# Vincentqyw/image-matching-webui

Measured on AMD Instinct MI355X. Metric: image-pairs/sec @640x480 SuperPoint+LightGlue, higher is better.
Workload: dtype f32 via 3xf16 split MFMA, f32 accumulate; P.V of LightGlue's cross blocks in two products (audited per block: layer error <= 7.1e-6, score error <= 4.7e-5, profiles/r05_lab_attention_mix.txt)

## Files before the change

image-matching-webui_amd/csrc/gemm_wreg.hip:

```cpp
#include <stdlib.h>

#include "gemm.h"
#include "gemm_tile.h"

#define WR_BN 256
#ifdef WR_LAB
__device__ int wr_lab_flags = 0;
#define WR_FLAGS (__builtin_amdgcn_readfirstlane(wr_lab_flags))
#else
#define WR_FLAGS 0
#endif
#define WR_F_NOSTORE 1
#define WR_F_ONETILE 2
#define WR_F_NOEPI 4
#define WR_F_NOWLOAD 8
#define WR_F_NOXLOAD 16
#define WR_F_NOSTORE_V 32
#define WR_F_NOSTORE_QK 64
#define WR_F_STAGGER(f) (((f) >> 8) & 255)
#define WR_STG_ROW 68
#define WR_STG_TROW 36
#define WR_WAVE_LDS 9216

typedef unsigned int u32x4_t __attribute__((ext_vector_type(4)));
__device__ __forceinline__ const void* wr_uniform_ptr(const void* p) {
    const size_t v = (size_t)p;
    const unsigned lo32 = (unsigned)__builtin_amdgcn_readfirstlane((int)(unsigned)(v & 0xffffffffu));
    const unsigned hi32 = (unsigned)__builtin_amdgcn_readfirstlane((int)(unsigned)(v >> 32));
    return (const void*)((size_t)lo32 | ((size_t)hi32 << 32));
}
__device__ __forceinline__ void wr_wave_fence() {
    __builtin_amdgcn_s_waitcnt(0xc07f);
    __builtin_amdgcn_wave_barrier();
}

template <int EPI, bool SINGLE, bool PIPE = true, int MT = 4>
__global__ __launch_bounds__(256, 2) void gemm_wreg_kernel(GemmP p) {
    __shared__ uint4 smem[(4 * WR_WAVE_LDS) / 16];
    char* sm = reinterpret_cast<char*>(smem);
    const int tid = threadIdx.x;
    const int lane = tid & 63, wid = tid >> 6;
    const int lo = lane & 31, hi = lane >> 5;
    TileCtx c;
    if (!gemm_tile_setup(p, c, WR_BN, 32 * MT)) return;
    const float* A = p.A + (size_t)c.z * p.a_bs;
    const float wsc = p.wscale ? p.wscale[c.wsel] : 1.0f;
    const int labf = WR_FLAGS;
    if (WR_F_STAGGER(labf) != 0 && (int)blockIdx.x >= p.st_nct && (int)blockIdx.x < 4 * p.st_nct)
        for (int i = 0; i < WR_F_STAGGER(labf) * ((int)blockIdx.x / p.st_nct); ++i) __builtin_amdgcn_s_sleep(16);
    const int nkt = (labf & WR_F_ONETILE) ? 1 : p.K >> 5, nks = 2 * nkt;

    f32x16 acc[2][MT];
#pragma unroll
    for (int n = 0; n < 2; ++n)
#pragma unroll
        for (int m = 0; m < MT; ++m)
#pragma unroll
            for (int r = 0; r < 16; ++r) acc[n][m][r] = 0.0f;

    const int g = tid & 3;
    const int rl0 = tid >> 2, rl1 = 64 + (tid >> 2);
    const bool st0 = MT >= 2 || rl0 < 32, st1 = MT == 4;
    const int wo0 = (((g >> 1) * 4 + (rl0 >> 5)) * 64 + (g & 1) * 32 + ((rl0 & 31) ^ (2 * g))) * 16;
    const int wo1 = (((g >> 1) * 4 + (rl1 >> 5)) * 64 + (g & 1) * 32 + ((rl1 & 31) ^ (2 * g))) * 16;
    const float* pa0 = A + (size_t)min(c.row0 + (st0 ? rl0 : 0), c.M - 1) * p.lda + g * 8;
    const float* pa1 = A + (size_t)min(c.row0 + (st1 ? rl1 : 0), c.M - 1) * p.lda + g * 8;
    bool lnc = false;
    float mu0 = 0.f, mu1 = 0.f;
    if constexpr (EPI == EPI_QKV_VIT || EPI == EPI_CONV) {
        lnc = p.ln_stats != nullptr;
        if (lnc) {
            mu0 = p.ln_stats[2 * (size_t)min(c.row0 + (st0 ? rl0 : 0), c.M - 1)];
            mu1 = p.ln_stats[2 * (size_t)min(c.row0 + (st1 ? rl1 : 0), c.M - 1)];
        }
    }
    f32x4 xa0, xb0, xa1, xb1;
    auto issue = [&](int kt) __attribute__((always_inline)) {
        if (st0) {
            xa0 = *reinterpret_cast<const f32x4*>(pa0 + kt * 32);
            xb0 = *reinterpret_cast<const f32x4*>(pa0 + kt * 32 + 4);
        }
        if (st1) {
            xa1 = *reinterpret_cast<const f32x4*>(pa1 + kt * 32);
            xb1 = *reinterpret_cast<const f32x4*>(pa1 + kt * 32 + 4);
        }
    };
    auto store = [&](int stg) __attribute__((always_inline)) {
        uint4 h, l;
        if constexpr (EPI == EPI_QKV_VIT || EPI == EPI_CONV) {
            if (lnc) {
                xa0 -= mu0;
                xb0 -= mu0;
                xa1 -= mu1;
                xb1 -= mu1;
            }
        }
        if constexpr (SINGLE) {
            if (st0) *reinterpret_cast<uint4*>(sm + stg * 16384 + wo0) = half8_rtn(__builtin_bit_cast(float4, xa0), __builtin_bit_cast(float4, xb0));
            if (st1) *reinterpret_cast<uint4*>(sm + stg * 16384 + wo1) = half8_rtn(__builtin_bit_cast(float4, xa1), __builtin_bit_cast(float4, xb1));
            return;
        }
        if (st0) {
            split8(__builtin_bit_cast(float4, xa0), __builtin_bit_cast(float4, xb0), h, l);
            *reinterpret_cast<uint4*>(sm + stg * 16384 + wo0) = h;
            if constexpr (!SINGLE) *reinterpret_cast<uint4*>(sm + stg * 16384 + 8192 + wo0) = l;
        }
        if (st1) {
            split8(__builtin_bit_cast(float4, xa1), __builtin_bit_cast(float4, xb1), h, l);
            *reinterpret_cast<uint4*>(sm + stg * 16384 + wo1) = h;
            if constexpr (!SINGLE) *reinterpret_cast<uint4*>(sm + stg * 16384 + 8192 + wo1) = l;
        }
    };
    const int nfr = (p.N + 31) >> 5;
    const size_t plane_bytes = (size_t)nfr * 32 * p.K * 2;
    const __amdgpu_buffer_rsrc_t rWh =
        __builtin_amdgcn_make_buffer_rsrc(const_cast<void*>(wr_uniform_ptr(p.Wh + (size_t)c.wsel * p.w_stride)), 0, (unsigned)plane_bytes, 0x00020000);
    const __amdgpu_buffer_rsrc_t rWl =
        __builtin_amdgcn_make_buffer_rsrc(const_cast<void*>(wr_uniform_ptr(p.Wl + (size_t)c.wsel * p.w_stride)), 0, (unsigned)plane_bytes, 0x00020000);
    unsigned wof[2];
#pragma unroll
    for (int n = 0; n < 2; ++n) {
        const int nf = min((c.col0 >> 5) + 2 * wid + n, nfr - 1);
        wof[n] = (unsigned)((nf * (p.K >> 4)) * 64 + lane) * 16u;
    }
    uint4 wc[2][2], wn[2][2];
    auto loadw = [&](int s, uint4(&w)[2][2]) __attribute__((always_inline)) {
#pragma unroll
        for (int n = 0; n < 2; ++n) {
            const u32x4_t vh = __builtin_amdgcn_raw_buffer_load_b128(rWh, wof[n], (unsigned)s * 1024u, 0);
            w[n][0] = make_uint4(vh.x, vh.y, vh.z, vh.w);
            if constexpr (!SINGLE) {
                const u32x4_t vl = __builtin_amdgcn_raw_buffer_load_b128(rWl, wof[n], (unsigned)s * 1024u, 0);
                w[n][1] = make_uint4(vl.x, vl.y, vl.z, vl.w);
            }
        }
    };
    auto kstep = [&](int stg, int ks, uint4(&w)[2][2]) __attribute__((always_inline)) {
        const int apos = (hi * 32 + (lo ^ (2 * (2 * ks + hi)))) * 16;
#pragma unroll
        for (int mh = 0; mh < (MT + 1) / 2; ++mh) {
            constexpr int MH = MT >= 2 ? 2 : 1;
            uint4 ah[MH], al[MH];
#pragma unroll
            for (int m = 0; m < MH; ++m) {
                const int fo = stg * 16384 + (ks * 4 + 2 * mh + m) * 1024 + apos;
                ah[m] = *reinterpret_cast<const uint4*>(sm + fo);
                if constexpr (!SINGLE) al[m] = *reinterpret_cast<const uint4*>(sm + fo + 8192);
            }
#pragma unroll
            for (int n = 0; n < 2; ++n)
#pragma unroll
                for (int m = 0; m < MH; ++m) {
                    if constexpr (!SINGLE) {
                        acc[n][2 * mh + m] = mfma16(w[n][0], al[m], acc[n][2 * mh + m]);
                        acc[n][2 * mh + m] = mfma16(w[n][1], ah[m], acc[n][2 * mh + m]);
                    }
                    acc[n][2 * mh + m] = mfma16(w[n][0], ah[m], acc[n][2 * mh + m]);
                }
            if constexpr (PIPE) {
                if (mh == 0) __builtin_amdgcn_sched_barrier(0);
            }
        }
    };

    if constexpr (PIPE) {
        uint4 w0[2][2], w1[2][2], w2[2][2];
        issue(0);
        loadw(0, w0);
        if (nks > 1) loadw(1, w1);
        store(0);
        if (nkt > 1) issue(1);
        __syncthreads();
#define WR_TILE(KT, WA, WB, WC)                                  \
    {                                                            \
        const int kt_ = (KT), stg_ = kt_ & 1, s_ = 2 * kt_;      \
        if (s_ + 2 < nks && !(labf & WR_F_NOWLOAD)) loadw(s_ + 2, WC); \
        __builtin_amdgcn_sched_barrier(0);                       \
        kstep(stg_, 0, WA);                                      \
        __builtin_amdgcn_sched_barrier(0);                       \
        if (kt_ + 1 < nkt && !(labf & WR_F_NOXLOAD)) {           \
            store(stg_ ^ 1);                                     \
            if (kt_ + 2 < nkt) issue(kt_ + 2);                   \
        }                                                        \
        if (s_ + 3 < nks && !(labf & WR_F_NOWLOAD)) loadw(s_ + 3, WA); \
        __builtin_amdgcn_sched_barrier(0);                       \
        kstep(stg_, 1, WB);                                      \
        __syncthreads();                                         \
    }
        int kt = 0;
#pragma unroll 1
        for (; kt + 3 <= nkt; kt += 3) {
            WR_TILE(kt, w0, w1, w2)
            WR_TILE(kt + 1, w2, w0, w1)
            WR_TILE(kt + 2, w1, w2, w0)
        }
        if (kt < nkt) WR_TILE(kt, w0, w1, w2)
        if (kt + 1 < nkt) WR_TILE(kt + 1, w2, w0, w1)
#undef WR_TILE
    } else {
    issue(0);
    loadw(0, wc);
    store(0);
    if (nkt > 1) issue(1);
    __syncthreads();
#pragma unroll 1
    for (int kt = 0; kt < nkt; ++kt) {
        const int stg = kt & 1;
        loadw(2 * kt + 1, wn);
        kstep(stg, 0, wc);
        if (kt + 1 < nkt) {
            store(stg ^ 1);
            if (kt + 2 < nkt) issue(kt + 2);
            loadw(2 * kt + 2, wc);
        }
        kstep(stg, 1, wn);
        __syncthreads();
    }
    }

    float* st = reinterpret_cast<float*>(sm + wid * WR_WAVE_LDS);
    const int fw0 = c.col0 + 64 * wid;
    if (fw0 >= c.N) return;
    if (labf & WR_F_NOEPI) {
        if (acc[0][0][0] == 12345.678f) p.C[0] = acc[1][MT - 1][3];
        return;
    }
    bool do_store = !(labf & WR_F_NOSTORE);
    auto park_rows = [&](int m) __attribute__((always_inline)) {
#pragma unroll
        for (int n = 0; n < 2; ++n)
#pragma unroll
            for (int q = 0; q < 4; ++q)
                *reinterpret_cast<float4*>(st + lo * WR_STG_ROW + 32 * n + 8 * q + 4 * hi) =
                    make_float4(acc[n][m][4 * q + 0] * wsc, acc[n][m][4 * q + 1] * wsc, acc[n][m][4 * q + 2] * wsc, acc[n][m][4 * q + 3] * wsc);
    };
    if constexpr (EPI == EPI_QKV || EPI == EPI_CROSS || EPI == EPI_QKV_VIT) {
        const int CW = p.heads * 64;
        const int t = fw0 / CW, hd = (fw0 - t * CW) >> 6;
        float* dst;
        bool vt, rope, scale;
        if (EPI == EPI_QKV || EPI == EPI_QKV_VIT) {
            const int role = t + (EPI == EPI_QKV_VIT ? p.role0 : 0);
            dst = (role == 0) ? p.Q : (role == 1) ? p.Kt : p.V;
            vt = (role == 2);
            rope = (role < 2);
            scale = (role == 0);
        } else {
            dst = (t == 0) ? p.Q : p.V;
            vt = (t == 1);
            rope = false;
            scale = (t == 0);
        }
        unsigned short* d16 = reinterpret_cast<unsigned short*>(dst);
        if ((labf & WR_F_NOSTORE_V) && vt) do_store = false;
        if ((labf & WR_F_NOSTORE_QK) && !vt) do_store = false;
        const int R = p.rows_per_seq;
        const int i0 = c.row0 - c.seq * R;
        if (EPI == EPI_QKV_VIT && !vt) {
            const int tab0 = i0 + (p.rope_seq_row0 ? p.rope_seq_row0[c.seq] : 0);
            const int d0 = (lane & 7) * 8, dp = d0 ^ 16;
            const bool first = (d0 & 16) == 0;
            const int ti = (d0 >> 5) * 16 + (d0 & 8);
            float4 ba = make_float4(0.f, 0.f, 0.f, 0.f), bb = ba, pa = ba, pb = ba;
            if (c.bias != nullptr) {
                ba = *reinterpret_cast<const float4*>(c.bias + fw0 + d0);
                bb = *reinterpret_cast<const float4*>(c.bias + fw0 + d0 + 4);
                pa = *reinterpret_cast<const float4*>(c.bias + fw0 + dp);
                pb = *reinterpret_cast<const float4*>(c.bias + fw0 + dp + 4);
            }
#pragma unroll
            for (int m = 0; m < MT; ++m) {
                float4 tc[4][2], ts[4][2];
#pragma unroll
                for (int pass = 0; pass < 4; ++pass) {
                    const size_t ir = (size_t)(tab0 + 32 * m + pass * 8 + (lane >> 3)) * 32 + ti;
                    tc[pass][0] = *reinterpret_cast<const float4*>(p.rope_cos + ir);
                    tc[pass][1] = *reinterpret_cast<const float4*>(p.rope_cos + ir + 4);
                    ts[pass][0] = *reinterpret_cast<const float4*>(p.rope_sin + ir);
                    ts[pass][1] = *reinterpret_cast<const float4*>(p.rope_sin + ir + 4);
                }
                park_rows(m);
                wr_wave_fence();
#pragma unroll
                for (int pass = 0; pass < 4; ++pass) {
                    const int tl = pass * 8 + (lane >> 3);
                    const float4 va = *reinterpret_cast<const float4*>(st + tl * WR_STG_ROW + d0);
                    const float4 vb = *reinterpret_cast<const float4*>(st + tl * WR_STG_ROW + d0 + 4);
                    const float4 wa = *reinterpret_cast<const float4*>(st + tl * WR_STG_ROW + dp);
                    const float4 wb = *reinterpret_cast<const float4*>(st + tl * WR_STG_ROW + dp + 4);
                    float mine[8] = {va.x + ba.x, va.y + ba.y, va.z + ba.z, va.w + ba.w, vb.x + bb.x, vb.y + bb.y, vb.z + bb.z, vb.w + bb.w};
                    float part[8] = {wa.x + pa.x, wa.y + pa.y, wa.z + pa.z, wa.w + pa.w, wb.x + pb.x, wb.y + pb.y, wb.z + pb.z, wb.w + pb.w};
                    if (lnc) {
                        const float2 mr = *reinterpret_cast<const float2*>(p.ln_stats + 2 * (size_t)(c.row0 + 32 * m + tl));
                        const float xa[8] = {va.x, va.y, va.z, va.w, vb.x, vb.y, vb.z, vb.w}, xp[8] = {wa.x, wa.y, wa.z, wa.w, wb.x, wb.y, wb.z, wb.w};
                        const float ba8[8] = {ba.x, ba.y, ba.z, ba.w, bb.x, bb.y, bb.z, bb.w}, pa8[8] = {pa.x, pa.y, pa.z, pa.w, pb.x, pb.y, pb.z, pb.w};
#pragma unroll
                        for (int j = 0; j < 8; ++j) {
                            mine[j] = mr.y * xa[j] + ba8[j];
                            part[j] = mr.y * xp[j] + pa8[j];
                        }
                    }
                    const float cw[8] = {tc[pass][0].x, tc[pass][0].y, tc[pass][0].z, tc[pass][0].w, tc[pass][1].x, tc[pass][1].y, tc[pass][1].z, tc[pass][1].w};
                    const float ss[8] = {ts[pass][0].x, ts[pass][0].y, ts[pass][0].z, ts[pass][0].w, ts[pass][1].x, ts[pass][1].y, ts[pass][1].z, ts[pass][1].w};
                    float v[8];
#pragma unroll
                    for (int j = 0; j < 8; ++j) {
                        float x = mine[j], y = part[j];
                        asm volatile("" : "+v"(x), "+v"(y));
                        const float r = first ? __builtin_fmaf(x, cw[j], -(y * ss[j])) : __builtin_fmaf(x, cw[j], y * ss[j]);
                        v[j] = scale ? r * p.alpha : r;
                    }
                    uint4 hv, lv;
                    split8(make_float4(v[0], v[1], v[2], v[3]), make_float4(v[4], v[5], v[6], v[7]), hv, lv);
                    unsigned short* o = d16 + (((size_t)c.seq * p.heads + hd) * R + i0 + 32 * m + tl) * 64 + d0;
                    if (do_store) {
                        *reinterpret_cast<uint4*>(o) = hv;
                        *reinterpret_cast<uint4*>(o + p.plane_halves) = lv;
                    }
                }
                wr_wave_fence();
            }
        } else if (!vt) {
            const int d0 = (lane & 7) * 8;
            float4 ba = make_float4(0.f, 0.f, 0.f, 0.f), bb = ba;
            if (c.bias != nullptr) {
                ba = *reinterpret_cast<const float4*>(c.bias + fw0 + d0);
                bb = *reinterpret_cast<const float4*>(c.bias + fw0 + d0 + 4);
            }
            float4 tc[2][4], ts[2][4];
            auto load_tables = [&](int m, float4(&cs)[4], float4(&sn)[4]) __attribute__((always_inline)) {
#pragma unroll
                for (int pass = 0; pass < 4; ++pass) {
                    const size_t row = (size_t)(c.row0 + 32 * m + pass * 8 + (lane >> 3));
                    cs[pass] = *reinterpret_cast<const float4*>(p.rope_cos + row * 32 + (d0 >> 1));
                    sn[pass] = *reinterpret_cast<const float4*>(p.rope_sin + row * 32 + (d0 >> 1));
                }
            };
            if (rope) load_tables(0, tc[0], ts[0]);
#pragma unroll
            for (int m = 0; m < MT; ++m) {
                park_rows(m);
                wr_wave_fence();
                if (rope && m + 1 < MT) load_tables(m + 1, tc[(m + 1) & 1], ts[(m + 1) & 1]);
#pragma unroll
                for (int pass = 0; pass < 4; ++pass) {
                    const int tl = pass * 8 + (lane >> 3);
                    const float4 va = *reinterpret_cast<const float4*>(st + tl * WR_STG_ROW + d0);
                    const float4 vb = *reinterpret_cast<const float4*>(st + tl * WR_STG_ROW + d0 + 4);
                    float v[8] = {va.x + ba.x, va.y + ba.y, va.z + ba.z, va.w + ba.w, vb.x + bb.x, vb.y + bb.y, vb.z + bb.z, vb.w + bb.w};
                    if (rope) {
                        const float4 cs = tc[m & 1][pass], sn = ts[m & 1][pass];
                        const float cw[4] = {cs.x, cs.y, cs.z, cs.w}, ss[4] = {sn.x, sn.y, sn.z, sn.w};
#pragma unroll
                        for (int j = 0; j < 4; ++j) {
                            float a0 = v[2 * j], a1 = v[2 * j + 1];
                            asm volatile("" : "+v"(a0), "+v"(a1));
                            v[2 * j] = __builtin_fmaf(a0, cw[j], -(a1 * ss[j]));
                            v[2 * j + 1] = __builtin_fmaf(a1, cw[j], a0 * ss[j]);
                        }
                    }
                    if (scale) {
#pragma unroll
                        for (int j = 0; j < 8; ++j) v[j] *= p.alpha;
                    }
                    uint4 hv, lv;
                    split8(make_float4(v[0], v[1], v[2], v[3]), make_float4(v[4], v[5], v[6], v[7]), hv, lv);
                    unsigned short* o = d16 + (((size_t)c.seq * p.heads + hd) * R + i0 + 32 * m + tl) * 64 + d0;
                    if (do_store) {
                        *reinterpret_cast<uint4*>(o) = hv;
                        *reinterpret_cast<uint4*>(o + p.plane_halves) = lv;
                    }
                }
                wr_wave_fence();
            }
        } else {
#pragma unroll
            for (int m = 0; m < MT; ++m) {
#pragma unroll
                for (int n = 0; n < 2; ++n)
#pragma unroll
                    for (int r = 0; r < 16; ++r) st[(32 * n + 8 * (r >> 2) + 4 * hi + (r & 3)) * WR_STG_TROW + lo] = acc[n][m][r] * wsc;
                wr_wave_fence();
#pragma unroll
                for (int pass = 0; pass < 4; ++pass) {
                    const int d = pass * 16 + (lane >> 2), tk = (lane & 3) * 8;
                    const float bd = c.bias ? c.bias[fw0 + d] : 0.0f;
                    float4 va = *reinterpret_cast<const float4*>(st + d * WR_STG_TROW + tk);
                    float4 vb = *reinterpret_cast<const float4*>(st + d * WR_STG_TROW + tk + 4);
                    if (lnc) {
                        const float4* ms4 = reinterpret_cast<const float4*>(p.ln_stats + 2 * (size_t)(c.row0 + 32 * m + tk));
                        const float4 q0 = ms4[0], q1 = ms4[1], q2 = ms4[2], q3 = ms4[3];
                        va = make_float4(q0.y * va.x, q0.w * va.y, q1.y * va.z, q1.w * va.w);
                        vb = make_float4(q2.y * vb.x, q2.w * vb.y, q3.y * vb.z, q3.w * vb.w);
                    }
                    uint4 hv, lv;
                    split8(make_float4(va.x + bd, va.y + bd, va.z + bd, va.w + bd), make_float4(vb.x + bd, vb.y + bd, vb.z + bd, vb.w + bd), hv, lv);
                    unsigned short* o = d16 + (((size_t)c.seq * p.heads + hd) * 64 + d) * R + i0 + 32 * m + tk;
                    if (do_store) {
                        *reinterpret_cast<uint4*>(o) = hv;
                        *reinterpret_cast<uint4*>(o + p.plane_halves) = lv;
                    }
                }
                wr_wave_fence();
            }
        }
    } else {
        float* C = p.C + (size_t)c.z * p.c_bs;
        const int fl = (lane & 15) * 4;
        const int f0 = fw0 + fl;
        float4 b4 = make_float4(0.f, 0.f, 0.f, 0.f);
        if (c.bias != nullptr) b4 = *reinterpret_cast<const float4*>(c.bias + f0);
#pragma unroll
        for (int m = 0; m < MT; ++m) {
            park_rows(m);
            wr_wave_fence();
#pragma unroll
            for (int pass = 0; pass < 8; ++pass) {
                const int tl = pass * 4 + (lane >> 4);
                const int row = c.row0 + 32 * m + tl;
                if (row < c.M) {
                    float4 t4 = *reinterpret_cast<const float4*>(st + tl * WR_STG_ROW + fl);
                    if (lnc) {
                        const float rs = p.ln_stats[2 * (size_t)row + 1];
                        t4 = make_float4(rs * t4.x, rs * t4.y, rs * t4.z, rs * t4.w);
                    }
                    float v[4] = {t4.x + b4.x, t4.y + b4.y, t4.z + b4.z, t4.w + b4.w};
                    float* dstp = C + (size_t)row * p.ldc + f0;
                    if (EPI == EPI_CONV) {
                        if (p.resid != nullptr) {
                            const float4 r4 = *reinterpret_cast<const float4*>(p.resid + (size_t)row * p.ldr + f0);
                            v[0] += r4.x;
                            v[1] += r4.y;
                            v[2] += r4.z;
                            v[3] += r4.w;
                        }
                        if (p.act == 1) {
#pragma unroll
                            for (int j = 0; j < 4; ++j) v[j] = fmaxf(v[j], 0.0f);
                        } else if (p.act == 2) {
#pragma unroll
                            for (int j = 0; j < 4; ++j) v[j] = v[j] > 0.0f ? v[j] : 0.01f * v[j];
                        } else if (p.act == 3) {
#pragma unroll
                            for (int j = 0; j < 4; ++j) v[j] = gelu_poly(v[j]);
                        }
                    } else if (EPI == EPI_BIAS) {
#pragma unroll
                        for (int j = 0; j < 4; ++j) v[j] *= p.alpha;
                    } else if (EPI == EPI_RELU) {
#pragma unroll
                        for (int j = 0; j < 4; ++j) v[j] = fmaxf(v[j], 0.0f);
                    } else if (EPI == EPI_RESID) {
                        const float4 o4 = *reinterpret_cast<const float4*>(dstp);
                        v[0] += o4.x;
                        v[1] += o4.y;
                        v[2] += o4.z;
                        v[3] += o4.w;
                    }
                    if (do_store) *reinterpret_cast<float4*>(dstp) = make_float4(v[0], v[1], v[2], v[3]);
                }
            }
            wr_wave_fence();
        }
    }
}

bool gemm_wreg_ok(const imcui_hip_s* h, const GemmP& p) {
    const int mode = h ? h->opt[OPT_GEMM_WREG] : 2;
    if (mode == 0 || (mode == 1 && p.epi != EPI_QKV && p.epi != EPI_CROSS && p.epi != EPI_QKV_VIT) || p.Wh == nullptr || p.Wl == nullptr || p.A2 != nullptr || p.conv_k > 0 || p.batch != 1 || p.mcnt || p.ncnt || p.group_rows > 1 ||
        p.rup_h > 0)
        return false;
    if (p.K % 32 != 0 || p.N % 64 != 0 || (p.lda & 3) != 0) return false;
    if (p.ln_stats != nullptr && p.epi != EPI_QKV_VIT && p.epi != EPI_CONV) return false;
    if (p.epi == EPI_QKV_VIT)
        return p.split_out && p.v_transposed && p.heads % 4 == 0 && p.N % (p.heads * 64) == 0 && p.rows_per_seq > 0 && p.rows_per_seq % 128 == 0 && p.M % 128 == 0 && !p.single;
    if (p.epi == EPI_QKV || p.epi == EPI_CROSS)
        return p.split_out && p.v_transposed && p.heads == 4 && p.N % 256 == 0 && p.rows_per_seq > 0 && p.rows_per_seq % 128 == 0 && p.M % 128 == 0;
    if (p.single && p.epi != EPI_CONV) return false;
    if ((p.ldc & 3) != 0 || (p.epi == EPI_CONV && p.resid != nullptr && (p.ldr & 3) != 0)) return false;
    return p.epi == EPI_BIAS || p.epi == EPI_RELU || p.epi == EPI_RESID || p.epi == EPI_CONV;
}

template <int EPI, int MT>
static void wreg_launch_small(imcui_hip_s* h, const GemmP& p, hipStream_t stream) {
    gemm_route_note(h, MT == 2 ? GR_WREG_MT2 : GR_WREG_MT1, EPI);
    hipLaunchKernelGGL((gemm_wreg_kernel<EPI, false, true, MT>), dim3(cdiv(p.M, 32 * MT) * cdiv(p.N, WR_BN), 1, 1), dim3(256), 0, stream, p);
}
static int wreg_tile_tokens(const imcui_hip_s* h, const GemmP& p) {
    if (p.epi != EPI_QKV && p.epi != EPI_CROSS && p.epi != EPI_BIAS && p.epi != EPI_CONV) return 128;
    if (p.single || p.group_rows > 1 || (h && h->opt[OPT_WREG_PIPE] == 0)) return 128;
    const int forced = h ? h->opt[OPT_WREG_TILE] : 0;
    if (forced == 128 || forced == 64 || forced == 32) return forced;
    const long ncol = cdiv(p.N, WR_BN);
    if ((long)cdiv(p.M, 128) * ncol >= 256) return 128;
    if ((long)cdiv(p.M, 64) * ncol >= 256) return 64;
    return 32;
}
template <bool PIPE>
static void wreg_launch(imcui_hip_s* h, const GemmP& p, hipStream_t stream) {
    const dim3 grid(cdiv(p.M, BM) * cdiv(p.N, WR_BN), 1, 1);
    const int kind = PIPE ? GR_WREG_PIPE : GR_WREG_ROLLED;
    switch (p.epi) {
        case EPI_BIAS: gemm_route_note(h, kind, EPI_BIAS); hipLaunchKernelGGL((gemm_wreg_kernel<EPI_BIAS, false, PIPE>), grid, dim3(256), 0, stream, p); break;
        case EPI_RELU: gemm_route_note(h, kind, EPI_RELU); hipLaunchKernelGGL((gemm_wreg_kernel<EPI_RELU, false, PIPE>), grid, dim3(256), 0, stream, p); break;
        case EPI_RESID: gemm_route_note(h, kind, EPI_RESID); hipLaunchKernelGGL((gemm_wreg_kernel<EPI_RESID, false, PIPE>), grid, dim3(256), 0, stream, p); break;
        case EPI_QKV: gemm_route_note(h, kind, EPI_QKV); hipLaunchKernelGGL((gemm_wreg_kernel<EPI_QKV, false, PIPE>), grid, dim3(256), 0, stream, p); break;
        case EPI_CROSS: gemm_route_note(h, kind, EPI_CROSS); hipLaunchKernelGGL((gemm_wreg_kernel<EPI_CROSS, false, PIPE>), grid, dim3(256), 0, stream, p); break;
        case EPI_QKV_VIT: gemm_route_note(h, kind, EPI_QKV_VIT); hipLaunchKernelGGL((gemm_wreg_kernel<EPI_QKV_VIT, false, PIPE>), grid, dim3(256), 0, stream, p); break;
        default:
            if (p.single) {
                gemm_route_note(h, PIPE ? GR_WREG_PIPE_SINGLE : GR_WREG_ROLLED_SINGLE, EPI_CONV);
                hipLaunchKernelGGL((gemm_wreg_kernel<EPI_CONV, true, PIPE>), grid, dim3(256), 0, stream, p);
            } else {
                gemm_route_note(h, kind, EPI_CONV);
                hipLaunchKernelGGL((gemm_wreg_kernel<EPI_CONV, false, PIPE>), grid, dim3(256), 0, stream, p);
            }
    }
}
void gemm_wreg_launch(imcui_hip_s* h, const GemmP& p, hipStream_t stream) {
    const int tok = wreg_tile_tokens(h, p);
    if (tok != 128) {
        if (p.epi == EPI_QKV)
            tok == 64 ? wreg_launch_small<EPI_QKV, 2>(h, p, stream) : wreg_launch_small<EPI_QKV, 1>(h, p, stream);
        else if (p.epi == EPI_CROSS)
            tok == 64 ? wreg_launch_small<EPI_CROSS, 2>(h, p, stream) : wreg_launch_small<EPI_CROSS, 1>(h, p, stream);
        else if (p.epi == EPI_CONV)
            tok == 64 ? wreg_launch_small<EPI_CONV, 2>(h, p, stream) : wreg_launch_small<EPI_CONV, 1>(h, p, stream);
        else
            tok == 64 ? wreg_launch_small<EPI_BIAS, 2>(h, p, stream) : wreg_launch_small<EPI_BIAS, 1>(h, p, stream);
        return;
    }
    if (h && h->opt[OPT_WREG_PIPE] == 0)
        wreg_launch<false>(h, p, stream);
    else
        wreg_launch<true>(h, p, stream);
}
```

Measured before the change: 980.6.

## Restage transposed V epilogue over multiple M steps per n-half for wider stores

The transposed V-plane epilogue now stages accumulators for one 32-column n-half across several M sub-tiles at once (WR_VT_STEPS, default 2). Each lane therefore writes longer contiguous runs along the token axis, and bias loads are hoisted per n-half. A lane-dependent swizzle for the VM=4 case targets LDS bank conflicts. The per-wave LDS footprint can grow for plane epilogues, which may reduce occupancy; ln_stats loads are shared per group.

```diff
diff --git a/image-matching-webui_amd/csrc/gemm_wreg.hip b/image-matching-webui_amd/csrc/gemm_wreg.hip
--- a/image-matching-webui_amd/csrc/gemm_wreg.hip
+++ b/image-matching-webui_amd/csrc/gemm_wreg.hip
@@ -19,8 +19,11 @@
 #define WR_F_NOSTORE_QK 64
 #define WR_F_STAGGER(f) (((f) >> 8) & 255)
 #define WR_STG_ROW 68
-#define WR_STG_TROW 36
 #define WR_WAVE_LDS 9216
+#ifndef WR_VT_STEPS
+#define WR_VT_STEPS 2
+#endif
+#define WR_VT_LDS(steps) (32 * (32 * (steps) + 4) * 4)
 
 typedef unsigned int u32x4_t __attribute__((ext_vector_type(4)));
 __device__ __forceinline__ const void* wr_uniform_ptr(const void* p) {
@@ -36,7 +39,10 @@
 
 template <int EPI, bool SINGLE, bool PIPE = true, int MT = 4>
 __global__ __launch_bounds__(256, 2) void gemm_wreg_kernel(GemmP p) {
-    __shared__ uint4 smem[(4 * WR_WAVE_LDS) / 16];
+    constexpr bool PLANES = EPI == EPI_QKV || EPI == EPI_CROSS || EPI == EPI_QKV_VIT;
+    constexpr int VM = MT < WR_VT_STEPS ? MT : WR_VT_STEPS;
+    constexpr int WAVE_LDS = PLANES && WR_VT_LDS(VM) > WR_WAVE_LDS ? WR_VT_LDS(VM) : WR_WAVE_LDS;
+    __shared__ uint4 smem[(4 * WAVE_LDS) / 16];
     char* sm = reinterpret_cast<char*>(smem);
     const int tid = threadIdx.x;
     const int lane = tid & 63, wid = tid >> 6;
@@ -218,7 +224,7 @@
     }
     }
 
-    float* st = reinterpret_cast<float*>(sm + wid * WR_WAVE_LDS);
+    float* st = reinterpret_cast<float*>(sm + wid * WAVE_LDS);
     const int fw0 = c.col0 + 64 * wid;
     if (fw0 >= c.N) return;
     if (labf & WR_F_NOEPI) {
@@ -374,34 +380,51 @@
                 wr_wave_fence();
             }
         } else {
-#pragma unroll
-            for (int m = 0; m < MT; ++m) {
-#pragma unroll
-                for (int n = 0; n < 2; ++n)
-#pragma unroll
-                    for (int r = 0; r < 16; ++r) st[(32 * n + 8 * (r >> 2) + 4 * hi + (r & 3)) * WR_STG_TROW + lo] = acc[n][m][r] * wsc;
-                wr_wave_fence();
-#pragma unroll
-                for (int pass = 0; pass < 4; ++pass) {
-                    const int d = pass * 16 + (lane >> 2), tk = (lane & 3) * 8;
-                    const float bd = c.bias ? c.bias[fw0 + d] : 0.0f;
-                    float4 va = *reinterpret_cast<const float4*>(st + d * WR_STG_TROW + tk);
-                    float4 vb = *reinterpret_cast<const float4*>(st + d * WR_STG_TROW + tk + 4);
+            constexpr int TROW = 32 * VM + 4;
+            constexpr int LPR = 4 * VM;
+            constexpr int RPP = 64 / LPR;
+            constexpr int NP = 32 / RPP;
+            const int dl = lane / LPR, tk = (lane % LPR) * 8;
+            const int sw = (VM == 4 && (lane & 8)) ? 4 : 0;
+#pragma unroll
+            for (int n = 0; n < 2; ++n) {
+                float bd[NP];
+#pragma unroll
+                for (int pass = 0; pass < NP; ++pass) bd[pass] = c.bias ? c.bias[fw0 + 32 * n + pass * RPP + dl] : 0.0f;
+#pragma unroll
+                for (int mg = 0; mg < MT; mg += VM) {
+                    float4 q0 = make_float4(0.f, 0.f, 0.f, 0.f), q1 = q0, q2 = q0, q3 = q0;
                     if (lnc) {
-                        const float4* ms4 = reinterpret_cast<const float4*>(p.ln_stats + 2 * (size_t)(c.row0 + 32 * m + tk));
-                        const float4 q0 = ms4[0], q1 = ms4[1], q2 = ms4[2], q3 = ms4[3];
-                        va = make_float4(q0.y * va.x, q0.w * va.y, q1.y * va.z, q1.w * va.w);
-                        vb = make_float4(q2.y * vb.x, q2.w * vb.y, q3.y * vb.z, q3.w * vb.w);
-                    }
-                    uint4 hv, lv;
-                    split8(make_float4(va.x + bd, va.y + bd, va.z + bd, va.w + bd), make_float4(vb.x + bd, vb.y + bd, vb.z + bd, vb.w + bd), hv, lv);
-                    unsigned short* o = d16 + (((size_t)c.seq * p.heads + hd) * 64 + d) * R + i0 + 32 * m + tk;
-                    if (do_store) {
-                        *reinterpret_cast<uint4*>(o) = hv;
-                        *reinterpret_cast<uint4*>(o + p.plane_halves) = lv;
-                    }
-                }
-                wr_wave_fence();
+                        const float4* ms4 = reinterpret_cast<const float4*>(p.ln_stats + 2 * (size_t)(c.row0 + 32 * mg + tk));
+                        q0 = ms4[0], q1 = ms4[1], q2 = ms4[2], q3 = ms4[3];
+                    }
+#pragma unroll
+                    for (int mm = 0; mm < VM; ++mm) {
+#pragma unroll
+                        for (int r = 0; r < 16; ++r) st[(8 * (r >> 2) + 4 * hi + (r & 3)) * TROW + 32 * mm + lo] = acc[n][mg + mm][r] * wsc;
+                    }
+                    wr_wave_fence();
+#pragma unroll
+                    for (int pass = 0; pass < NP; ++pass) {
+                        const int d = pass * RPP + dl;
+                        const float4 x0 = *reinterpret_cast<const float4*>(st + d * TROW + tk + sw);
+                        const float4 x1 = *reinterpret_cast<const float4*>(st + d * TROW + tk + (sw ^ 4));
+                        float4 va = sw ? x1 : x0, vb = sw ? x0 : x1;
+                        if (lnc) {
+                            va = make_float4(q0.y * va.x, q0.w * va.y, q1.y * va.z, q1.w * va.w);
+                            vb = make_float4(q2.y * vb.x, q2.w * vb.y, q3.y * vb.z, q3.w * vb.w);
+                        }
+                        const float b1 = bd[pass];
+                        uint4 hv, lv;
+                        split8(make_float4(va.x + b1, va.y + b1, va.z + b1, va.w + b1), make_float4(vb.x + b1, vb.y + b1, vb.z + b1, vb.w + b1), hv, lv);
+                        unsigned short* o = d16 + (((size_t)c.seq * p.heads + hd) * 64 + 32 * n + d) * R + i0 + 32 * mg + tk;
+                        if (do_store) {
+                            *reinterpret_cast<uint4*>(o) = hv;
+                            *reinterpret_cast<uint4*>(o + p.plane_halves) = lv;
+                        }
+                    }
+                    wr_wave_fence();
+                }
             }
         }
     } else {
```

After: 986.7, median of 6. About the same (+0.6%).
